# sunhui-3D/3D-PointCloudReconstruction

Measured on NVIDIA B200. Metric: chamfer_fwd_bwd_point_pairs_per_s, higher is better.
Workload: dtype f32

## Files before the change

### 3d-pointcloudreconstruction_b200/_lib.py

```python
import ctypes
import os

import torch

_HERE = os.path.dirname(os.path.abspath(__file__))
LIB_PATH = os.environ.get("PSD_B200_LIB") or os.path.join(_HERE, "libpsd_b200.so")

if not os.path.exists(LIB_PATH):
    raise ImportError(
        f"{LIB_PATH} is missing: build it with `python 3d-pointcloudreconstruction_b200/build.py` "
        "(nvcc, sm_100a). This package has no CPU or eager fallback."
    )

lib = ctypes.CDLL(LIB_PATH)

_vp = ctypes.c_void_p
_ci = ctypes.c_int
_cf = ctypes.c_float

_SIGNATURES = {
    "psd_chamfer_forward": [_vp, _vp, _ci, _ci, _ci, _vp, _vp, _vp, _vp, _vp],
    "psd_chamfer_forward_ex": [_vp, _vp, _ci, _ci, _ci, _ci, _vp, _vp, _vp, _vp, _vp, _cf, _vp, _ci, _ci, _vp],
    "psd_chamfer_forward_zero": [_vp, _vp, _ci, _ci, _ci, _ci, _vp, _vp, _vp, _vp, _vp, _cf, _vp, _vp, ctypes.c_longlong, _vp],
    "psd_chamfer_backward": [_vp] * 8 + [_ci, _ci, _ci, _vp],
# ... 8 lines not shown
    "psd_chamfer_forward_host": [_vp, _vp, _ci, _ci, _ci, _vp, _vp, _vp, _vp, _vp],
    "psd_fp32_fma_peak": [_cf, ctypes.POINTER(_cf), _vp],
    "psd_chamfer_stats": [ctypes.POINTER(ctypes.c_longlong), _ci],
    "psd_chamfer_nn_variant": [_ci],
    "psd_chamfer_mean_loss_forward": [_vp, _vp, _ci, _ci, _ci, _ci, _vp, _vp, _vp, _vp, _vp, _vp, _vp],
    "psd_chamfer_mean_loss_forward_zero": [_vp, _vp, _ci, _ci, _ci, _ci, _vp, _vp, _vp, _vp, _vp, _vp, _vp, ctypes.c_longlong, _vp],
    "psd_chamfer_mean_loss_backward": [_vp, _vp, _vp, _vp, _vp, _vp, _vp, _ci, _ci, _ci, _vp],
    "psd_chamfer_mean_loss_backward_ex": [_vp, _vp, _vp, _vp, _vp, _vp, _vp, _ci, _ci, _ci, _ci, _ci, _vp],
    "psd_chamfer_loss_step_host": [_vp, _vp, _ci, _ci, _ci, _vp, _vp, _vp, _vp, _vp, _vp],
    "psd_chamfer_loss_step_host_ex": [_vp, _vp, _ci, _ci, _ci, _vp, _vp, _vp, _vp, _vp, _ci, _ci, _vp],
    "psd_chamfer_loss_step_pred_dev": [_vp, _ci, _vp, _ci, _ci, _ci, _vp, _vp, _ci, _ci, _vp],
    "psd_host_step_graphs": [_ci],
    "psd_emd_solo_mode": [_ci],
    "psd_emd_grid_mode": [_ci],
    "psd_chamfer_tc_ctas": [_ci],
    "psd_proj_min_dist": [_vp, _vp, _vp, _ci, _ci, _ci, _ci, _vp, _vp, _vp],
    "psd_icp_batch": [_vp, _vp, _ci, _ci, _ci, _vp, _ci, ctypes.c_double, _vp, _vp, _vp, _vp],
    "psd_nn_f64": [_vp, _vp, _ci, _ci, _ci, _ci, _vp, _vp, _vp],
    "psd_farthest_point_sample": [_vp, _ci, _ci, _ci, _ci, _vp, _vp],
    "psd_cont_proj": [_vp, _ci, _ci, _ci, _ci, ctypes.c_float, _vp, _vp],
    "psd_cont_proj_backward": [_vp, _vp, _ci, _ci, _ci, _ci, ctypes.c_float, _vp, _vp],
    "psd_debug_tc_prof": [_vp],
    "psd_debug_tc_filter": [_vp, _vp, _ci, _ci, _ci, _vp, _vp, _vp, _vp, _vp, _ci, _vp],
}
lib.psd_version.restype = _ci
lib.psd_last_error.restype = ctypes.c_char_p
for _n, _a in _SIGNATURES.items():
    getattr(lib, _n).argtypes = _a
    getattr(lib, _n).restype = _ci

# ... 32 lines not shown
```

### 3d-pointcloudreconstruction_b200/csrc/chamfer.cu

```cuda
#include "chamfer_nn.cuh"
#include "psd_device.h"

#ifndef PSD_GRAD_TRIGGER_EARLY
#define PSD_GRAD_TRIGGER_EARLY 1
#endif
namespace psd {

constexpr int kWarps = 16;
constexpr int kThreads = kWarps * 32;
constexpr int kPartBytes = kWarps * kQB * 12;

__device__ unsigned long long g_fallback_queries = 0ull;

struct BlockInfo {
    int blk, d, cloud, qblock;
    float cx, cy, cz;
    float t2max;
    int bad;
    int pad[3];
};
constexpr int kPerBlockBytes = kPartBytes + (int)sizeof(BlockInfo) + 3 * kQB * 4 + kQB * 4;

template <int TM>
__global__ void __launch_bounds__(kThreads, 1) chamfer_nn_kernel(const NNParams p) {
// ... 546 lines not shown
        D.q_bs = 3LL * nq; D.t_bs = 3LL * nt;
        int qb0 = q_begin < 0 ? 0 : q_begin;
        if (qb0 > nq) qb0 = nq;
        int qc = (q_count < 0) ? nq - qb0 : q_count;
        if (qb0 + qc > nq) qc = nq - qb0;
        D.q_begin = qb0; D.q_count = qc;
        D.qblocks = (qc + QB - 1) / QB;
        D.ntt = 1; D.ws = nullptr;
    };
    fill(p.dir[0], xyz1, n, 1, xyz2, m, 2, dist1, idx1, 0);
    fill(p.dir[1], xyz2, m, 2, xyz1, n, 1, dist2, idx2, 1);
    const long long blocks = (long long)b * (p.dir[0].qblocks + p.dir[1].qblocks);
    if (blocks == 0) return only_zero();
    if (blocks > 0x3fffffffLL) return cudaErrorInvalidConfiguration;
    p.zero_buf = zero_buf; p.zero_floats = zero_floats;
    p.pdl_trigger = 0;
    p.blocks_dir0 = b * p.dir[0].qblocks;
    p.total_blocks = (int)blocks;
    p.sums = sums; p.fs_count = fs_count; p.fs_thr = fs_thr;
    p.tile = 0; p.flush = 0;
    const int variant = g_nn_variant.load();
    if ((variant == 3 || (variant == 0 && blocks >= 2LL * num_sms)) && psd_nn_tc_supported(p)) {
        float *dbg = g_tc_dbg.exchange(nullptr);
        return psd_launch_nn_tc(p, ds, stream, dbg, g_tc_dbg_ld.load(), g_tc_prof.load(), b);
    }
    const int grid = blocks < num_sms ? (int)blocks : num_sms;
    const int per_cta = (int)((blocks + grid - 1) / grid);
    int tile = 1024;
    const int tmax = n > m ? n : m;
    while (tile < tmax && tile < 4096) tile *= 2;
    const size_t fixed = (size_t)tile * 16 + 2048;
// ... 70 lines not shown
```

### 3d-pointcloudreconstruction_b200/csrc/chamfer_nn.cuh

```cuda
#pragma once
#include "psd_common.cuh"

namespace psd {

constexpr int kQ = 4;
constexpr int kQB = 32 * kQ;
constexpr int kChunk = 16;
constexpr float kBig = 1e30f;
constexpr float kLimit = 1e18f;
constexpr int kRefTile = 512;

struct NNDirection {
    const float *q;
    const float *t;
    long long q_ps, q_cs, q_bs;
    long long t_ps, t_cs, t_bs;
    float *dist;
    int *idx;
    int nq, nt;
    int q_begin, q_count;
    int qblocks;
    int slot;
    int ntt;
    unsigned long long *ws;
};

struct NNParams {
    NNDirection dir[2];
    int blocks_dir0;
    int total_blocks;
    int tile;
    int flush;
    float *sums;
    int *fs_count;
    float fs_thr;
    float *zero_buf;
    long long zero_floats;
    int pdl_trigger;
};

__device__ __forceinline__ void zero_fill(const NNParams &p) {
    if (p.zero_buf == nullptr) return;
    const long long nth = (long long)gridDim.x * blockDim.x, t0 = (long long)blockIdx.x * blockDim.x + threadIdx.x;
    if (((reinterpret_cast<unsigned long long>(p.zero_buf) & 15ull) == 0ull) && (p.zero_floats & 3) == 0) {
        float4 *z = reinterpret_cast<float4 *>(p.zero_buf);
        for (long long i = t0; i < (p.zero_floats >> 2); i += nth) z[i] = make_float4(0.f, 0.f, 0.f, 0.f);
    } else {
        for (long long i = t0; i < p.zero_floats; i += nth) p.zero_buf[i] = 0.f;
    }
}

__device__ __forceinline__ float exact_d(const float *__restrict__ tb, long long tps, long long tcs, int k, float x1,
                                         float y1, float z1) {
// ... 6 lines not shown
```

### 3d-pointcloudreconstruction_b200/csrc/chamfer_nn_tc.cu

```cuda
#include <cuda_fp16.h>
#include "chamfer_nn.cuh"
#include "psd_device.h"

namespace psd {
namespace tc {

#ifndef PSD_TC_SCAN_WARPS
#define PSD_TC_SCAN_WARPS 8
#endif
#ifndef PSD_TC_SETMAXNREG
#define PSD_TC_SETMAXNREG (PSD_TC_SCAN_WARPS == 16)
#endif
#ifndef PSD_TC_STAGE_FIRST
#define PSD_TC_STAGE_FIRST 0
#endif
#ifndef PSD_TC_TAIL_FAST
#define PSD_TC_TAIL_FAST 1
#endif
#ifndef PSD_TC_ALT_UNROLL
#define PSD_TC_ALT_UNROLL 2
#endif
#ifndef PSD_TC_SCAN_ALT
#define PSD_TC_SCAN_ALT 1
#endif
// ... 23 lines not shown
constexpr int kMaxT = 2048;
constexpr float kPadW = 32768.0f;
constexpr float kQMax = 4096.0f;

constexpr int kOffB = 0;
constexpr int kOffA = kOffB + 2 * kBRows * 32;
constexpr int kOffRaw = kOffA + 2 * kQB * 32;
constexpr int kOffPart = kOffRaw + 2 * 3 * kMaxT * 4;
constexpr int kOffSq = kOffPart + 2 * kColGroups * 3 * kQB * 4;
constexpr int kFbCap = 512;
constexpr int kOffFb = kOffSq + 3 * 3 * kQB * 4;
constexpr int kOffFq = kOffFb + kFbCap * 4;
constexpr int kOffStat = kOffFq + 3 * kFbCap * 4;
constexpr int kOffBar = kOffStat + 3 * 32 * 4 + 16;
constexpr int kOffMisc = kOffBar + 16 * 8;
constexpr int kSmemTC = kOffMisc + 64;
static_assert(kOffBar % 8 == 0 && kOffA % 128 == 0 && kOffRaw % 16 == 0 && kOffPart % 16 == 0 && kHelpWarps <= 8 && kThreadsTC / 32 <= 32 &&
              kSmemTC <= 227 * 1024, "shared-memory carve-up");

__device__ unsigned long long g_fallback_queries_tc = 0ull;

__device__ __forceinline__ uint32_t smem_u32(const void *p) { return (uint32_t)__cvta_generic_to_shared(p); }
__device__ __forceinline__ void mbar_init(uint32_t bar, uint32_t count) {
    asm volatile("mbarrier.init.shared::cta.b64 [%0], %1;" ::"r"(bar), "r"(count) : "memory");
}
__device__ __forceinline__ void mbar_arrive(uint32_t bar) {
    asm volatile("mbarrier.arrive.shared::cta.b64 _, [%0];" ::"r"(bar) : "memory");
}
__device__ __forceinline__ uint32_t mbar_try_wait(uint32_t bar, uint32_t parity) {
    uint32_t ok;
    asm volatile("{ .reg .pred p; mbarrier.try_wait.parity.shared::cta.b64 p, [%1], %2; selp.u32 %0, 1, 0, p; }"
                 : "=r"(ok) : "r"(bar), "r"(parity) : "memory");
    return ok;
// ... 41 lines not shown
        __syncwarp();
    } else if (PSD_TC_SPIN & 2) {
        mbar_spin(bar, parity, abort_flag);
    } else {
        mbar_wait(bar, parity, abort_flag);
    }
}
__device__ __forceinline__ void cp_async4(void *smem_dst, const float *gsrc) {
    asm volatile("cp.async.ca.shared.global [%0], [%1], 4;" ::"r"(smem_u32(smem_dst)), "l"(gsrc) : "memory");
}
__device__ __forceinline__ void cp_async_wait_all() { asm volatile("cp.async.wait_all;" ::: "memory"); }
__device__ __forceinline__ void tc_fence_before() { asm volatile("tcgen05.fence::before_thread_sync;" ::: "memory"); }
__device__ __forceinline__ void tc_fence_after() { asm volatile("tcgen05.fence::after_thread_sync;" ::: "memory"); }
__device__ __forceinline__ void fence_async_smem() { asm volatile("fence.proxy.async.shared::cta;" ::: "memory"); }
__device__ __forceinline__ void help_bar() { asm volatile("bar.sync 1, %0;" ::"n"(kHelpThreads) : "memory"); }
__device__ __forceinline__ void split_h(float x, unsigned short &hi, unsigned short &lo) {
    const __half h = __float2half_rn(x);
    const __half l = __float2half_rn(x - __half2float(h));
    hi = __half_as_ushort(h); lo = __half_as_ushort(l);
}
__device__ __forceinline__ void split_h2(float a, float b, unsigned short &ah, unsigned short &al, unsigned short &bh, unsigned short &bl) {
    const __half2 h = __floats2half2_rn(a, b);
    const float2 hf = __half22float2(h);
    const __half2 l = __floats2half2_rn(a - hf.x, b - hf.y);
    ah = __half_as_ushort(__low2half(h)); bh = __half_as_ushort(__high2half(h));
    al = __half_as_ushort(__low2half(l)); bl = __half_as_ushort(__high2half(l));
}
__device__ __forceinline__ uint32_t pack2(unsigned short a, unsigned short b) { return (uint32_t)a | ((uint32_t)b << 16); }
__device__ __forceinline__ uint64_t umma_desc(uint32_t saddr) {
    return (uint64_t)((saddr & 0x3ffffu) >> 4) | ((uint64_t)(128u >> 4) << 16) | ((uint64_t)(256u >> 4) << 32) |
// ... 77 lines not shown
}
__device__ __forceinline__ int group_of(const NNParams &p, const Unit &u) { return u.d * 0x40000000 + u.cloud * p.dir[u.d].ntt + u.ttile; }
__device__ __forceinline__ const float *targets_of(const NNParams &p, const Unit &u) {
    const NNDirection &D = p.dir[u.d];
    return D.t + (long long)u.cloud * D.t_bs + (long long)u.t0 * D.t_ps;
}
__device__ __forceinline__ void store_result(const NNDirection &D, const Unit &u, int j, float dist, int idx_local) {
    if (D.ws) atomicMin(D.ws + (long long)u.cloud * D.nq + j, pack_key(dist, u.t0 + idx_local));
    else { D.dist[(long long)u.cloud * D.nq + j] = dist; D.idx[(long long)u.cloud * D.nq + j] = u.t0 + idx_local; }
}

struct Frame {
    float cx, cy, cz, cs, wmax;
    int bad, bsel;
};

struct FbQuery {
    Unit u;
    int j, nt, res;
    float x1, y1, z1;
    bool nan_possible;
    const float *bx, *by, *bz;
    long long ps;
};
__device__ __forceinline__ FbQuery fallback_query(const NNParams &p, int blk_begin, int e, const float *sraw, const int *s_rawgroup,
                                                  const float *fq) {
    FbQuery q;
    q.u = decode_unit(p, blk_begin + ((e & 0x3fffffff) >> 8));
    const NNDirection &D = p.dir[q.u.d];
    q.nt = q.u.nt;
// ... 82 lines not shown
    float *sraw = reinterpret_cast<float *>(smem + kOffRaw);
    float *part = reinterpret_cast<float *>(smem + kOffPart);
    float *sq = reinterpret_cast<float *>(smem + kOffSq);
    int *fb_list = reinterpret_cast<int *>(smem + kOffFb);
    float *fb_q = reinterpret_cast<float *>(smem + kOffFq);
    int *s_nfb = reinterpret_cast<int *>(smem + kOffMisc) + 1;
    float *s_wstat = reinterpret_cast<float *>(smem + kOffStat);
    int *s_bstat = reinterpret_cast<int *>(smem + kOffStat) + 32;
    float *s_cstat = reinterpret_cast<float *>(smem + kOffStat) + 64;
    int *s_rawgroup = reinterpret_cast<int *>(smem + kOffStat) + 96;
    uint32_t *s_tmem = reinterpret_cast<uint32_t *>(smem + kOffMisc);
    volatile int *s_abort = reinterpret_cast<volatile int *>(smem + kOffMisc) + 2;
    const uint32_t sB_addr = smem_u32(smem + kOffB), sA_addr = smem_u32(smem + kOffA);
    const uint32_t bar0 = smem_u32(smem + kOffBar);
    const uint32_t bar_full = bar0, bar_empty = bar0 + 8 * kBufs, bar_ready = bar0 + 16 * kBufs, bar_part = bar_ready + 16;

    const int tid = threadIdx.x, lane = tid & 31, warp = tid >> 5;
    const int G = gridDim.x;
    const int blk_begin = (int)(((long long)blockIdx.x * p.total_blocks) / G);
    const int blk_end = (int)(((long long)(blockIdx.x + 1) * p.total_blocks) / G);
    const int nunits = blk_end - blk_begin;
    long long *pf = (DBG && prof) ? prof + (long long)blockIdx.x * 64 : nullptr;
    auto stamp = [&](int slot) { if (DBG && pf && slot < 56) pf[slot] = clock64(); };
    long long *tl = (DBG && prof && blockIdx.x == 0) ? prof + (long long)gridDim.x * 64 : nullptr;
    auto tstamp = [&](int rowi, int g) { if (DBG && tl && g < 64) tl[rowi * 64 + g] = clock64(); };
    if (tid == 0) stamp(0);

    if (tid == 0) {
        for (int i = 0; i < kBufs; ++i) { mbar_init(bar_full + 8 * i, 1); mbar_init(bar_empty + 8 * i, PSD_TC_SCAN_ALT ? 4 : kScanWarps); }
        for (int i = 0; i < 2; ++i) { mbar_init(bar_ready + 8 * i, 1); mbar_init(bar_part + 8 * i, kScanWarps); }
        *s_abort = 0;
        *s_nfb = 0;
        s_rawgroup[0] = -1; s_rawgroup[1] = -1;
        asm volatile("fence.mbarrier_init.release.cluster;" ::: "memory");
    }
    if (warp == kMmaWarp) {
        asm volatile("tcgen05.alloc.cta_group::1.sync.aligned.shared::cta.b32 [%0], %1;" ::"r"(smem_u32(s_tmem)), "r"(512u) : "memory");
        asm volatile("tcgen05.relinquish_alloc_permit.cta_group::1.sync.aligned;" ::: "memory");
    }
    tc_fence_before();
    __syncthreads();
    tc_fence_after();
    const uint32_t tmem_base = *s_tmem;
    if (tid == 0) stamp(1);
    pdl_wait();
    zero_fill(p);

    auto frame_of = [&](int nt, int bsel, int tt, int tn, int tw, auto &&team_bar, Frame &fr, int &bad) {
        const float *rx = sraw + (bsel * 3) * kMaxT, *ry = rx + kMaxT, *rz = ry + kMaxT;
        float cx, cy, cz;
        {
            float sx = 0.f, sy = 0.f, sz = 0.f;
            const int ns = nt < 8 ? nt : 8;
            const int step = nt >> 3;
#pragma unroll
            for (int s8 = 0; s8 < 8; ++s8) {
                if (s8 < ns) {
                    const int k = nt < 8 ? s8 : s8 * step;
// ... 64 lines not shown
    auto build_b = [&](int nt, int bsel, int tt, int tn, int tw, auto &&team_bar, Frame &fr) {
        int bad = 0;
        float wmax = 0.f;
        frame_of(nt, bsel, tt, tn, tw, team_bar, fr, bad);
        build_rows(nt, fr, 0, ((nt + kTileN - 1) / kTileN) * kTileN, tt, tn, wmax, bad);
        publish_stats(tw, wmax, bad);
    };
    auto pick_stats = [&](int nwarps, Frame &fr) {
        float wmax = 0.f;
        int bad = 0;
        for (int w = 0; w < nwarps; ++w) { wmax = fmaxf(wmax, s_wstat[w]); bad |= s_bstat[w]; }
        fr.wmax = wmax; fr.bad = bad;
    };

    Frame fr0 = {0.f, 0.f, 0.f, 1.f, 0.f, 0, 0};
    int group0 = -1;
    float pq1 = 0.f, pq2 = 0.f, pq3 = 0.f;
    if (nunits > 0) {
        const Unit u = decode_unit(p, blk_begin);
        const NNDirection &D = p.dir[u.d];
        group0 = group_of(p, u);
        const float *__restrict__ tb = targets_of(p, u);
#pragma unroll
        for (int comp = 0; comp < 3; ++comp)
            for (int k = tid; k < u.nt; k += kThreadsTC) cp_async4(sraw + comp * kMaxT + k, tb + k * D.t_ps + comp * D.t_cs);
        if (tid >= kHelp0 && tid - kHelp0 < kQB) {
            int j = D.q_begin + u.qblock * kQB + (tid - kHelp0);
            const int q_last = D.q_begin + D.q_count - 1;
            j = j < q_last ? j : q_last;
            const float *qp = D.q + (long long)u.cloud * D.q_bs + j * D.q_ps;
            pq1 = __ldg(qp); pq2 = __ldg(qp + D.q_cs); pq3 = __ldg(qp + 2 * D.q_cs);
        }
        if (tid == 0) stamp(6);
        cp_async_wait_all();
        __syncthreads();
        if (tid == 0) stamp(7);
        build_b(u.nt, 0, tid, kThreadsTC, warp, [] { __syncthreads(); }, fr0);
        fence_async_smem();
        __syncthreads();
        pick_stats(kThreadsTC / 32, fr0);
        if (tid == 0) s_rawgroup[0] = group0;
    }
    if (tid == 0) stamp(5);

    if (warp < kScanWarps) {
        if (PSD_TC_SETMAXNREG) asm volatile("setmaxnreg.dec.sync.aligned.u32 72;");
        const int r = warp & 3, c = warp >> 2;
        const int row = r * 32 + lane;
        const uint32_t tlane = tmem_base + ((uint32_t)(r * 32) << 16);
        int g0 = 0;
        long long a59 = 0;
        Unit u = decode_unit(p, blk_begin);
        for (int ul = 0; ul < nunits; ++ul) {
            if (ul > 0) advance_unit(p, u, blk_begin + ul);
            const int ntiles = (u.nt + kTileN - 1) / kTileN;
// ... 151 lines not shown
                    umma_commit(bar_full + 8 * b);
                    if (DBG) { const long long w3 = clock64(); a61 += w2 - w1; a62 += w3 - w2; if (tl && g < 64) tl[64 + g] = w3; }
                    bdesc += (uint64_t)((kTileN * 32) >> 4);
                }
            }
            if (DBG && pf) { pf[56] = a56; pf[57] = a57; pf[58] = clock64(); pf[61] = a61; pf[62] = a62; }
        }
        __syncwarp();
        if (PSD_TC_SETMAXNREG) asm volatile("setmaxnreg.dec.sync.aligned.u32 80;");
    } else {
        if (PSD_TC_SETMAXNREG) asm volatile("setmaxnreg.inc.sync.aligned.u32 96;");
        const int ht = tid - kHelp0, hw = warp - (kScanWarps + 1);
        int st_group = group0, st_bsel = 0;
        Frame fr_st = fr0;
        bool need_b = false;

        auto stage_changes_group = [&](const Unit &u) { return group_of(p, u) != st_group; };
        auto stage_issue = [&](int ul, const Unit &u) {
            const NNDirection &D = p.dir[u.d];
            if (ht < kQB && ul > 0) {
                int j = D.q_begin + u.qblock * kQB + ht;
                const int q_last = D.q_begin + D.q_count - 1;
                j = j < q_last ? j : q_last;
                const float *qp = D.q + (long long)u.cloud * D.q_bs + j * D.q_ps;
                pq1 = __ldg(qp); pq2 = __ldg(qp + D.q_cs); pq3 = __ldg(qp + 2 * D.q_cs);
            }
            const int group = group_of(p, u);
            need_b = group != st_group;
            if (need_b) {
                st_group = group;
                st_bsel ^= 1;
                const int nt = u.nt;
                const float *__restrict__ tb = targets_of(p, u);
                const long long tps = D.t_ps, tcs = D.t_cs;
                float *rx = sraw + (st_bsel * 3) * kMaxT;
#pragma unroll
                for (int comp = 0; comp < 3; ++comp)
                    for (int k = ht; k < nt; k += kHelpThreads) cp_async4(rx + comp * kMaxT + k, tb + k * tps + comp * tcs);
            }
        };
        auto stage_finish = [&](int ul, const Unit &u) {
            if (need_b) {
                cp_async_wait_all();
                help_bar();
                build_b(u.nt, st_bsel, ht, kHelpThreads, hw, [] { help_bar(); }, fr_st);
                if (ht == 0) s_rawgroup[st_bsel] = st_group;
            }
            if (ht < kQB) {
                float *sqp = sq + (ul % 3) * 3 * kQB;
                sqp[ht] = pq1; sqp[kQB + ht] = pq2; sqp[2 * kQB + ht] = pq3;
                const float sc = -2.0f * fr_st.cs;
                const float x = (pq1 - fr_st.cx) * sc, y = (pq2 - fr_st.cy) * sc, z = (pq3 - fr_st.cz) * sc;
                unsigned short xh, xl, yh, yl, zh, zl, uh, ul_;
                split_h2(x, y, xh, xl, yh, yl);
                split_h2(z, 0.f, zh, zl, uh, ul_);
                const unsigned short one = 0x3c00;
                unsigned char *dst = smem + kOffA + (ul & 1) * (kQB * 32) + (ht >> 3) * 256 + (ht & 7) * 16;
// ... 182 lines not shown
                const FbQuery q = fallback_query(p, blk_begin, fb_list[fi], sraw, s_rawgroup, fb_q + fi);
                const unsigned long long key = fallback_scan(q, item - fi * nsplit, nsplit, lane);
                if (lane == 0) atomicMin(s_keys + fi, key);
            }
            __syncthreads();
            for (int fi = tid; fi < nfb; fi += kThreadsTC) {
                const FbQuery q = fallback_query(p, blk_begin, fb_list[fi], sraw, s_rawgroup, fb_q + fi);
                fallback_write(p, q, s_keys[fi]);
            }
        }
        if (nfb > 0 && tid == 0) atomicAdd(&g_fallback_queries_tc, (unsigned long long)nfb);
    }
    if (tid == 0) stamp(4);
    if (warp == kMmaWarp)
        asm volatile("tcgen05.dealloc.cta_group::1.sync.aligned.b32 %0, %1;" ::"r"(tmem_base), "r"(512u) : "memory");
}

}
}

using namespace psd;

namespace psd {
namespace tc {
__global__ void __launch_bounds__(256) chamfer_nn_tc_finalize_kernel(const NNParams p, int b) {
    const long long n0 = p.dir[0].ws ? (long long)b * p.dir[0].q_count : 0;
    const long long n1 = p.dir[1].ws ? (long long)b * p.dir[1].q_count : 0;
    const long long gid = (long long)blockIdx.x * blockDim.x + threadIdx.x;
    const bool active = gid < n0 + n1;
    const int d = (active && gid >= n0) ? 1 : 0;
// ... 31 lines not shown
            if (p.sums) atomicAdd(p.sums + key2, ws);
            if (p.fs_count && wc) atomicAdd(p.fs_count + key2, wc);
        }
    }
}
}
}

bool psd_nn_tc_supported(const NNParams &p) {
    const long long t0 = (p.dir[0].nt + tc::kMaxT - 1) / tc::kMaxT, t1 = (p.dir[1].nt + tc::kMaxT - 1) / tc::kMaxT;
    return (long long)p.blocks_dir0 * t0 + (long long)(p.total_blocks - p.blocks_dir0) * t1 < 0x3fffffffLL;
}

static std::atomic<int> g_tc_max_ctas{0};
int psd_set_tc_max_ctas(int n) { return n >= 0 ? g_tc_max_ctas.exchange(n) : g_tc_max_ctas.load(); }

static cudaError_t acquire_merge_ws(DeviceState *ds, cudaStream_t stream, size_t elems, unsigned long long **out, bool *temp,
                                    MergeWorkspace **slot_out) {
    *temp = false; *slot_out = nullptr;
    cudaStreamCaptureStatus cap = cudaStreamCaptureStatusNone;
    cudaError_t e = cudaStreamIsCapturing(stream, &cap);
    if (e != cudaSuccess) return e;
    if (cap != cudaStreamCaptureStatusNone) {
        e = cudaMallocAsync(reinterpret_cast<void **>(out), elems * sizeof(unsigned long long), stream);
        if (e == cudaSuccess) e = cudaMemsetAsync(*out, 0xff, elems * sizeof(unsigned long long), stream);
        *temp = true;
        return e;
    }
    std::lock_guard<std::mutex> lock(state_mutex());
    MergeWorkspace *hit = nullptr, *victim = &ds->merge[0];
// ... 19 lines not shown
        if (e != cudaSuccess) { *w = MergeWorkspace(); return e; }
        w->elems = elems;
        w->dirty = true;
    }
    if (w->dirty) {
        e = cudaMemsetAsync(w->ptr, 0xff, w->elems * sizeof(unsigned long long), stream);
        if (e != cudaSuccess) return e;
        w->dirty = false;
    }
    w->used = true; w->stream = stream; w->last_use = ++ds->merge_clock;
    *out = w->ptr; *slot_out = w;
    return cudaSuccess;
}

cudaError_t psd_launch_nn_tc(const NNParams &p_in, DeviceState *ds, cudaStream_t stream, float *dbg, int dbg_ld, long long *prof, int b) {
    {
        std::lock_guard<std::mutex> lock(state_mutex());
        if (!ds->attr_tc) {
            cudaError_t e = cudaFuncSetAttribute(tc::chamfer_nn_tc_kernel<false>, cudaFuncAttributeMaxDynamicSharedMemorySize, tc::kSmemTC);
            if (e == cudaSuccess) e = cudaFuncSetAttribute(tc::chamfer_nn_tc_kernel<true>, cudaFuncAttributeMaxDynamicSharedMemorySize, tc::kSmemTC);
            if (e != cudaSuccess) return e;
            ds->attr_tc = true;
        }
    }
    NNParams p = p_in;
    unsigned long long *ws = nullptr;
    size_t ws_elems = 0;
    bool need_ws[2];
    for (int d = 0; d < 2; ++d) {
        p.dir[d].ntt = (p.dir[d].nt + tc::kMaxT - 1) / tc::kMaxT;
        need_ws[d] = p.dir[d].ntt > 1 && p.dir[d].q_count > 0;
        if (need_ws[d]) ws_elems += (size_t)b * p.dir[d].nq;
    }
    bool ws_temp = false;
    MergeWorkspace *ws_slot = nullptr;
    if (ws_elems) {
        cudaError_t e = acquire_merge_ws(ds, stream, ws_elems, &ws, &ws_temp, &ws_slot);
        if (e != cudaSuccess) return e;
    }
    {
        unsigned long long *w = ws;
        for (int d = 0; d < 2; ++d) {
            p.dir[d].ws = need_ws[d] ? w : nullptr;
            if (need_ws[d]) w += (size_t)b * p.dir[d].nq;
        }
    }
    const int blocks0 = p.blocks_dir0 * p.dir[0].ntt;
    const int blocks1 = (p.total_blocks - p.blocks_dir0) * p.dir[1].ntt;
    p.blocks_dir0 = blocks0;
    p.total_blocks = blocks0 + blocks1;
    int grid = p.total_blocks < ds->num_sms ? p.total_blocks : ds->num_sms;
    const int cap = g_tc_max_ctas.load();
    if (cap > 0 && grid > cap) grid = cap;
    p.pdl_trigger = (cap > 0 && grid == cap) ? 0 : 1;
    cudaError_t e;
    if (dbg || prof) e = psd_launch_pdl(p.pdl_trigger != 0, tc::chamfer_nn_tc_kernel<true>, dim3(grid), dim3(tc::kThreadsTC), tc::kSmemTC, stream, p, dbg, dbg_ld, prof);
    else e = psd_launch_pdl(p.pdl_trigger != 0, tc::chamfer_nn_tc_kernel<false>, dim3(grid), dim3(tc::kThreadsTC), tc::kSmemTC, stream, p, (float *)nullptr, 0, (long long *)nullptr);
    if (ws_elems) {
        if (e == cudaSuccess) {
            const long long total = (p.dir[0].ws ? (long long)b * p.dir[0].q_count : 0) + (p.dir[1].ws ? (long long)b * p.dir[1].q_count : 0);
            if (total > 0) {
                tc::chamfer_nn_tc_finalize_kernel<<<(unsigned)((total + 255) / 256), 256, 0, stream>>>(p, b);
                e = cudaGetLastError();
            }
        }
        if (ws_temp) {
            const cudaError_t e2 = cudaFreeAsync(ws, stream);
            if (e == cudaSuccess) e = e2;
        } else if (e != cudaSuccess && ws_slot) {
            std::lock_guard<std::mutex> lock(state_mutex());
            ws_slot->dirty = true;
        }
// ... 14 lines not shown
```

### 3d-pointcloudreconstruction_b200/csrc/psd_capi.cu

```cuda
#include <stdio.h>
#include <stdlib.h>
#include <string.h>

#include "../../include/psd_b200.h"
#include "psd_common.cuh"
#include "psd_device.h"

cudaError_t psd_launch_chamfer_forward(const float *xyz1, const float *xyz2, int b, int n, int m, int layout,
                                       float *dist1, float *dist2, int *idx1, int *idx2, float *sums, float fs_thr,
                                       int *fs_count, int q_begin, int q_count, cudaStream_t stream, float *zero_buf = nullptr,
                                       long long zero_floats = 0);
cudaError_t psd_launch_chamfer_backward(const float *xyz1, const float *xyz2, float *gradxyz1, float *gradxyz2,
                                        const float *graddist1, const float *graddist2, const int *idx1, const int *idx2,
                                        int b, int n, int m, int layout, int overwrite, cudaStream_t stream,
                                        const float *upstream = nullptr);
cudaError_t psd_launch_chamfer_mean_loss(const float *sums, int b, int n, int m, float *out, cudaStream_t stream);
cudaError_t psd_read_chamfer_stats(unsigned long long *fallback, int reset);
int psd_set_nn_variant(int v);
cudaError_t psd_launch_icp(const void *a, const void *b, int in_f64, int batch, int n, const double *init_pose, int max_iter,
                           double tol, double *T, double *dist, int *iters, cudaStream_t stream);
cudaError_t psd_launch_nn_f64(const void *src, const void *dst, int in_f64, int batch, int n_src, int n_dst, double *distances,
                              int *indices, cudaStream_t stream);
int psd_icp_max_points();
int psd_set_emd_solo(int enable);
int psd_set_emd_grid(int enable);
int psd_set_tc_max_ctas(int n);
cudaError_t psd_launch_cont_proj(const float *pcl, int b, int n, int grid_h, int grid_w, float sigma_sq, float *out,
                                 cudaStream_t stream);
cudaError_t psd_launch_cont_proj_backward(const float *pcl, const float *gout, int b, int n, int grid_h, int grid_w,
                                          float sigma_sq, float *gpcl, cudaStream_t stream);
cudaError_t psd_launch_fps(const float *xyz, int b, int n, int npoint, int start, long long *centroids, cudaStream_t stream);
int psd_fps_max_points();
cudaError_t psd_launch_proj_min_dist(const float *pred, const float *gt, const float *table, int b, int h, int w, int mode,
                                     float *out_min, float *out_inv, cudaStream_t stream);
void psd_set_tc_debug(float *dbg, int ld);
void psd_set_tc_prof(long long *prof);
cudaError_t psd_launch_emd_forward(const float *xyz1, const float *xyz2, int b, int n, float *dist, int *assignment,
                                   float *price, int *assignment_inv, int *bid, float *bid_increments,
                                   float *max_increments, float eps, int iters, int force_cluster, int fresh,
                                   float *loss_sums, cudaStream_t stream, int *unsupported);
cudaError_t psd_launch_emd_mean_loss(const float *sums, int b, int n, float *out, cudaStream_t stream);
// ... 248 lines not shown

int psd_nn_f64(const void *src, const void *dst, int in_f64, int batch, int n_src, int n_dst, double *distances, int *indices,
               void *stream) {
    if (batch < 0 || n_src < 0 || n_dst < 1) { psd_set_error_msg("psd_nn_f64: batch >= 0, n_src >= 0, n_dst >= 1 required"); return -1; }
    if ((size_t)n_dst * 24 > 200 * 1024) { psd_set_error_msg("psd_nn_f64: destination cloud too large for shared memory (n_dst <= 8533)"); return -1; }
    return finish("psd_nn_f64", psd_launch_nn_f64(src, dst, in_f64, batch, n_src, n_dst, distances, indices, (cudaStream_t)stream));
}

int psd_chamfer_nn_variant(int variant) { return psd_set_nn_variant(variant); }

int psd_emd_solo_mode(int enable) { return psd_set_emd_solo(enable); }

int psd_emd_grid_mode(int enable) { return psd_set_emd_grid(enable); }

int psd_chamfer_tc_ctas(int max_ctas) { return psd_set_tc_max_ctas(max_ctas); }

int psd_debug_tc_prof(long long *prof_dev) { psd_set_tc_prof(prof_dev); return 1; }

int psd_debug_tc_filter(const float *xyz1, const float *xyz2, int b, int n, int m, float *dist1, float *dist2, int *idx1,
                        int *idx2, float *dump, int dump_ld, void *stream) {
    const int old = psd_set_nn_variant(3);
    psd_set_tc_debug(dump, dump_ld);
    cudaError_t e = psd_launch_chamfer_forward(xyz1, xyz2, b, n, m, 0, dist1, dist2, idx1, idx2, nullptr, 0.f, nullptr, 0,
                                               -1, (cudaStream_t)stream);
    psd_set_tc_debug(nullptr, 0);
    psd_set_nn_variant(old);
    return finish("psd_debug_tc_filter", e);
}

int psd_chamfer_stats(long long *out_host2, int reset) {
// ... 73 lines not shown
    const bool own_g1 = (g1 == d_g1);
    if (!own_g1 && (e = cudaMemsetAsync(g1, 0, sizeof(float) * 3 * s1, stream)) != cudaSuccess) return e;
    e = psd_launch_chamfer_forward(x1, d_x2, b, n, m, layout, d_d1, d_d2, d_i1, d_i2, d_sums, 0.f, nullptr, 0, -1, stream,
                                   own_g1 ? d_g1 : d_g2, (long long)(own_g1 ? 3 * (s1 + s2) : 3 * s2));
    if (e == cudaSuccess) e = psd_launch_chamfer_mean_loss(d_sums, b, n, m, d_loss, stream);
    if (e == cudaSuccess) e = psd_launch_chamfer_backward(x1, d_x2, g1, d_g2, nullptr, nullptr, d_i1, d_i2, b, n, m, layout, 0, stream, nullptr);
    if (e != cudaSuccess) return e;
    e = cudaMemcpyAsync(a.loss_host, d_loss, sizeof(float), cudaMemcpyDeviceToHost, stream);
    if (e == cudaSuccess && a.g1_host) e = cudaMemcpyAsync(a.g1_host, g1, sizeof(float) * 3 * s1, cudaMemcpyDeviceToHost, stream);
    if (e == cudaSuccess && a.g2_host) e = cudaMemcpyAsync(a.g2_host, d_g2, sizeof(float) * 3 * s2, cudaMemcpyDeviceToHost, stream);
    return e;
}

struct StepGraph {
    const void *x1 = nullptr, *x2 = nullptr, *loss = nullptr, *g1 = nullptr, *g2 = nullptr, *g1u = nullptr, *ws = nullptr;
    int b = 0, n = 0, m = 0, variant = 0, device = -1, tc_ctas = 0, flags = 0;
    cudaGraphExec_t exec = nullptr;
    bool plain = false;
    unsigned long long last_use = 0;
    bool same(const StepGraph &o) const {
        return x1 == o.x1 && x2 == o.x2 && loss == o.loss && g1 == o.g1 && g2 == o.g2 && g1u == o.g1u && ws == o.ws && b == o.b &&
               n == o.n && m == o.m && variant == o.variant && device == o.device && tc_ctas == o.tc_ctas && flags == o.flags;
    }
};
static const int kStepGraphs = 64;
static StepGraph g_step_graph[kStepGraphs];
static unsigned long long g_step_clock = 0;
static int g_step_graph_enabled = -1;

static void drop_step_graphs(const void *ws) {
    for (StepGraph &g : g_step_graph)
        if (g.ws == ws) {
            if (g.exec) cudaGraphExecDestroy(g.exec);
            g = StepGraph();
        }
}

// ... 30 lines not shown
        ds->step_ws_bytes[slot] = need;
    }
    float *const ws = ds->step_ws[slot];
    if (gradxyz1_dev) *gradxyz1_dev = (a.x1_dev && a.g1_user) ? a.g1_user : ws + 3 * (s1 + s2);
    if (gradxyz2_dev) *gradxyz2_dev = ws + 3 * (s1 + s2) + 3 * s1;

    if (g_step_graph_enabled < 0) {
        const char *env = getenv("PSD_HOST_STEP_GRAPH");
        g_step_graph_enabled = (env && env[0] == '0') ? 0 : 1;
    }
    bool launched = false;
    if (g_step_graph_enabled && stream != nullptr && stream != cudaStreamLegacy) {
        StepGraph key;
        key.x1 = a.x1; key.x2 = a.x2; key.loss = a.loss_host; key.g1 = a.g1_host; key.g2 = a.g2_host; key.g1u = a.g1_user;
        key.ws = ws; key.b = b; key.n = n; key.m = m; key.variant = psd_set_nn_variant(-1); key.tc_ctas = psd_set_tc_max_ctas(-1);
        key.flags = (a.x1_dev ? 1 : 0) | (a.layout1 ? 2 : 0);
        key.device = ds->device;
        StepGraph *hit = nullptr, *victim = &g_step_graph[0];
        for (StepGraph &g : g_step_graph) {
            if (g.ws && g.same(key)) { hit = &g; break; }
            if (g.last_use < victim->last_use) victim = &g;
        }
        if (hit == nullptr) {
            if (victim->exec) cudaGraphExecDestroy(victim->exec);
            *victim = key;
            victim->last_use = ++g_step_clock;
        } else {
            hit->last_use = ++g_step_clock;
            if (hit->exec == nullptr && !hit->plain &&
                !((a.x1_dev || pinned_host(a.x1)) && pinned_host(a.x2) && pinned_host(a.loss_host) && pinned_host(a.g1_host) &&
// ... 113 lines not shown
```

### 3d-pointcloudreconstruction_b200/csrc/psd_common.cuh

```cuda
#pragma once
#include <cuda_runtime.h>
#include <stdint.h>

#if defined(__CUDA_ARCH__) && (__CUDA_ARCH__ < 1000)
#error "libpsd_b200 is written for sm_100a (B200) only"
#endif

namespace psd {

__device__ __forceinline__ float sqdist_exact(float dx, float dy, float dz) {
    return __fmaf_rn(dz, dz, __fmaf_rn(dx, dx, __fmul_rn(dy, dy)));
}

__device__ __forceinline__ float2 ffma2(float a, float2 b, float2 c) {
    return __ffma2_rn(make_float2(a, a), b, c);
}

__device__ __forceinline__ float fmin3(float a, float b, float c) {
    float d;
    asm("min.f32 %0, %1, %2, %3;" : "=f"(d) : "f"(a), "f"(b), "f"(c));
    return d;
}

#ifndef PSD_PDL
// ... 5 lines not shown
__device__ __forceinline__ void pdl_wait() {
    if (PSD_PDL) asm volatile("griddepcontrol.wait;" ::: "memory");
}

__device__ __forceinline__ unsigned long long pack_key(float d, int idx) {
    return ((unsigned long long)__float_as_uint(d) << 32) | (unsigned int)idx;
}

__device__ __forceinline__ unsigned long long shfl_xor_u64(unsigned long long v, int lane_mask) {
    return __shfl_xor_sync(0xffffffffu, v, lane_mask);
}

}

template <typename... KArgs, typename... Args>
static inline cudaError_t psd_launch_pdl(bool allow, void (*kernel)(KArgs...), dim3 grid, dim3 block, size_t smem, cudaStream_t stream, Args... args) {
    cudaLaunchConfig_t cfg = {};
    cfg.gridDim = grid; cfg.blockDim = block; cfg.dynamicSmemBytes = smem; cfg.stream = stream;
    cudaLaunchAttribute at[1];
    at[0].id = cudaLaunchAttributeProgrammaticStreamSerialization;
    at[0].val.programmaticStreamSerializationAllowed = (PSD_PDL && allow) ? 1 : 0;
    cfg.attrs = at; cfg.numAttrs = 1;
    return cudaLaunchKernelEx(&cfg, kernel, KArgs(args)...);
}

void psd_set_error(const char *what, cudaError_t err);
void psd_set_error_msg(const char *what);
```

### 3d-pointcloudreconstruction_b200/csrc/psd_device.h

```cpp
#pragma once
#include <cuda_runtime.h>

#include <atomic>
#include <mutex>

namespace psd {

constexpr int kMaxDevices = 64;
constexpr int kStepSlots = 8;
constexpr int kMergeSlots = 16;

struct MergeWorkspace {
    cudaStream_t stream = nullptr;
    unsigned long long *ptr = nullptr;
    size_t elems = 0;
    bool used = false;
    bool dirty = false;
    unsigned long long last_use = 0;
};

struct DeviceState {
    bool init = false;
    int device = -1;
    int num_sms = 0, max_smem = 0;
    bool attr_nn = false, attr_tc = false, attr_proj = false;
    float *fwd_ws = nullptr;
    size_t fwd_ws_bytes = 0;
    float *step_ws[kStepSlots] = {};
    size_t step_ws_bytes[kStepSlots] = {};
    MergeWorkspace merge[kMergeSlots];
    unsigned long long merge_clock = 0;
};

DeviceState *device_state(cudaError_t *err);
std::mutex &state_mutex();

}
```

### include/psd_b200.h

```cpp
#ifndef PSD_B200_H_
#define PSD_B200_H_

#ifdef __cplusplus
extern "C" {
#endif

int psd_version(void);

const char *psd_last_error(void);


int psd_chamfer_forward(const float *xyz1, const float *xyz2, int b, int n, int m, float *dist1, float *dist2,
                        int *idx1, int *idx2, void *stream);

int psd_chamfer_forward_ex(const float *xyz1, const float *xyz2, int b, int n, int m, int layout, float *dist1,
                           float *dist2, int *idx1, int *idx2, float *sums, float fs_thr, int *fs_count, int q_begin,
                           int q_count, void *stream);

int psd_chamfer_forward_zero(const float *xyz1, const float *xyz2, int b, int n, int m, int layout, float *dist1,
                             float *dist2, int *idx1, int *idx2, float *sums, float fs_thr, int *fs_count, float *zero_buf,
                             long long zero_floats, void *stream);

int psd_chamfer_backward(const float *xyz1, const float *xyz2, float *gradxyz1, float *gradxyz2,
                         const float *graddist1, const float *graddist2, const int *idx1, const int *idx2, int b, int n,
// ... 61 lines not shown
                                  int slot, int sync, void *stream);
int psd_chamfer_loss_step_pred_dev(const float *xyz1_dev, int layout1, const float *xyz2_host, int b, int n, int m,
                                   float *loss_host, float *gradxyz1_dev, int slot, int sync, void *stream);
int psd_host_step_graphs(int enable);


int psd_fp32_fma_peak(float ms_target, float *tflops, void *stream);

int psd_chamfer_stats(long long *out_host2, int reset);

int psd_chamfer_nn_variant(int variant);

int psd_emd_solo_mode(int enable);
int psd_emd_grid_mode(int enable);
int psd_chamfer_tc_ctas(int max_ctas);

int psd_debug_tc_filter(const float *xyz1, const float *xyz2, int b, int n, int m, float *dist1, float *dist2, int *idx1,
                        int *idx2, float *dump, int dump_ld, void *stream);

int psd_debug_tc_prof(long long *prof_dev);

#ifdef __cplusplus
}
#endif
#endif
```

Before: 7122 billion.

## Share target-tile B-operand builds between paired CTAs via 2-CTA clusters and DSMEM

Launches the tensor-core chamfer kernel as 2-CTA clusters. When a pair of CTAs each need the same two target groups at a group boundary, each CTA builds one group's split-half B operand and bulk-copies it, together with its frame, into the peer's shared memory through DSMEM with mbarrier transaction tracking. This is meant to remove duplicated target loads and B-operand construction at the start of each CTA's work range. In exchange it adds cluster barriers, a remote-arrive handshake before exit, and a cluster launch constraint that could limit occupancy. Pairing is on by default when the grid is even and enough clusters fit.

```diff
diff --git a/3d-pointcloudreconstruction_b200/_lib.py b/3d-pointcloudreconstruction_b200/_lib.py
--- a/3d-pointcloudreconstruction_b200/_lib.py
+++ b/3d-pointcloudreconstruction_b200/_lib.py
@@ -46,6 +46,7 @@
     "psd_emd_solo_mode": [_ci],
     "psd_emd_grid_mode": [_ci],
     "psd_chamfer_tc_ctas": [_ci],
+    "psd_chamfer_tc_pairs": [_ci],
     "psd_proj_min_dist": [_vp, _vp, _vp, _ci, _ci, _ci, _ci, _vp, _vp, _vp],
     "psd_icp_batch": [_vp, _vp, _ci, _ci, _ci, _vp, _ci, ctypes.c_double, _vp, _vp, _vp, _vp],
     "psd_nn_f64": [_vp, _vp, _ci, _ci, _ci, _ci, _vp, _vp, _vp],
diff --git a/3d-pointcloudreconstruction_b200/csrc/chamfer.cu b/3d-pointcloudreconstruction_b200/csrc/chamfer.cu
--- a/3d-pointcloudreconstruction_b200/csrc/chamfer.cu
+++ b/3d-pointcloudreconstruction_b200/csrc/chamfer.cu
@@ -584,7 +584,7 @@
     if (blocks == 0) return only_zero();
     if (blocks > 0x3fffffffLL) return cudaErrorInvalidConfiguration;
     p.zero_buf = zero_buf; p.zero_floats = zero_floats;
-    p.pdl_trigger = 0;
+    p.pdl_trigger = 0; p.pairs = 0;
     p.blocks_dir0 = b * p.dir[0].qblocks;
     p.total_blocks = (int)blocks;
     p.sums = sums; p.fs_count = fs_count; p.fs_thr = fs_thr;
diff --git a/3d-pointcloudreconstruction_b200/csrc/chamfer_nn.cuh b/3d-pointcloudreconstruction_b200/csrc/chamfer_nn.cuh
--- a/3d-pointcloudreconstruction_b200/csrc/chamfer_nn.cuh
+++ b/3d-pointcloudreconstruction_b200/csrc/chamfer_nn.cuh
@@ -37,6 +37,7 @@
     float *zero_buf;
     long long zero_floats;
     int pdl_trigger;
+    int pairs;
 };
 
 __device__ __forceinline__ void zero_fill(const NNParams &p) {
diff --git a/3d-pointcloudreconstruction_b200/csrc/chamfer_nn_tc.cu b/3d-pointcloudreconstruction_b200/csrc/chamfer_nn_tc.cu
--- a/3d-pointcloudreconstruction_b200/csrc/chamfer_nn_tc.cu
+++ b/3d-pointcloudreconstruction_b200/csrc/chamfer_nn_tc.cu
@@ -61,9 +61,10 @@
 constexpr int kOffStat = kOffFq + 3 * kFbCap * 4;
 constexpr int kOffBar = kOffStat + 3 * 32 * 4 + 16;
 constexpr int kOffMisc = kOffBar + 16 * 8;
+constexpr int kOffXFrame = kOffMisc + 16;
 constexpr int kSmemTC = kOffMisc + 64;
-static_assert(kOffBar % 8 == 0 && kOffA % 128 == 0 && kOffRaw % 16 == 0 && kOffPart % 16 == 0 && kHelpWarps <= 8 && kThreadsTC / 32 <= 32 &&
-              kSmemTC <= 227 * 1024, "shared-memory carve-up");
+static_assert(kOffBar % 8 == 0 && kOffA % 128 == 0 && kOffRaw % 16 == 0 && kOffPart % 16 == 0 && kOffXFrame % 16 == 0 &&
+              kHelpWarps <= 8 && kThreadsTC / 32 <= 32 && kSmemTC <= 227 * 1024, "shared-memory carve-up");
 
 __device__ unsigned long long g_fallback_queries_tc = 0ull;
 
@@ -135,6 +136,28 @@
 __device__ __forceinline__ void tc_fence_after() { asm volatile("tcgen05.fence::after_thread_sync;" ::: "memory"); }
 __device__ __forceinline__ void fence_async_smem() { asm volatile("fence.proxy.async.shared::cta;" ::: "memory"); }
 __device__ __forceinline__ void help_bar() { asm volatile("bar.sync 1, %0;" ::"n"(kHelpThreads) : "memory"); }
+__device__ __forceinline__ uint32_t cluster_rank() {
+    uint32_t r;
+    asm volatile("mov.u32 %0, %%cluster_ctarank;" : "=r"(r));
+    return r;
+}
+__device__ __forceinline__ uint32_t map_to_rank(uint32_t saddr, uint32_t rank) {
+    uint32_t r;
+    asm volatile("mapa.shared::cluster.u32 %0, %1, %2;" : "=r"(r) : "r"(saddr), "r"(rank));
+    return r;
+}
+__device__ __forceinline__ void cluster_arrive() { asm volatile("barrier.cluster.arrive.relaxed.aligned;" ::: "memory"); }
+__device__ __forceinline__ void cluster_wait() { asm volatile("barrier.cluster.wait.acquire.aligned;" ::: "memory"); }
+__device__ __forceinline__ void mbar_arrive_remote(uint32_t cluster_bar) {
+    asm volatile("mbarrier.arrive.release.cluster.shared::cluster.b64 _, [%0];" ::"r"(cluster_bar) : "memory");
+}
+__device__ __forceinline__ void mbar_expect_tx(uint32_t bar, uint32_t bytes) {
+    asm volatile("mbarrier.arrive.expect_tx.shared::cta.b64 _, [%0], %1;" ::"r"(bar), "r"(bytes) : "memory");
+}
+__device__ __forceinline__ void bulk_copy_to_cluster(uint32_t dst, uint32_t src, uint32_t bytes, uint32_t bar) {
+    asm volatile("cp.async.bulk.shared::cluster.shared::cta.mbarrier::complete_tx::bytes [%0], [%1], %2, [%3];"
+                 ::"r"(dst), "r"(src), "r"(bytes), "r"(bar) : "memory");
+}
 __device__ __forceinline__ void split_h(float x, unsigned short &hi, unsigned short &lo) {
     const __half h = __float2half_rn(x);
     const __half l = __float2half_rn(x - __half2float(h));
@@ -242,6 +265,34 @@
     float cx, cy, cz, cs, wmax;
     int bad, bsel;
 };
+
+struct PairPlan {
+    int role;
+    int buf;
+    int blk1;
+    uint32_t bytes;
+};
+__device__ __forceinline__ PairPlan pair_plan(const NNParams &p) {
+    PairPlan pl = {0, 0, 0, 0u};
+    if (!p.pairs) return pl;
+    const long long G = gridDim.x, lo = blockIdx.x & ~1u;
+    const int b0 = (int)((lo * p.total_blocks) / G), b1 = (int)(((lo + 1) * p.total_blocks) / G),
+              b2 = (int)(((lo + 2) * p.total_blocks) / G);
+    if (b0 == b1 || b1 == b2) return pl;
+    const Unit u0 = decode_unit(p, b0);
+    const int e1 = b0 + p.dir[u0.d].qblocks - u0.qblock;
+    if (e1 >= b2 || e1 == b1) return pl;
+    const Unit u1 = decode_unit(p, e1);
+    if (e1 + p.dir[u1.d].qblocks < b2) return pl;
+    const bool upper = (blockIdx.x & 1) != 0, lower_crosses = e1 < b1;
+    pl.role = upper == lower_crosses ? 1 : 2;
+    pl.buf = lower_crosses ? 1 : 0;
+    pl.blk1 = e1;
+    const int nt = lower_crosses ? u1.nt : u0.nt;
+    pl.bytes = (uint32_t)(((nt + kTileN - 1) / kTileN) * kTileN * 32 + 32);
+    return pl;
+}
+static_assert(sizeof(Frame) <= 32, "Frame slot");
 
 struct FbQuery {
     Unit u;
@@ -354,6 +405,9 @@
     const uint32_t sB_addr = smem_u32(smem + kOffB), sA_addr = smem_u32(smem + kOffA);
     const uint32_t bar0 = smem_u32(smem + kOffBar);
     const uint32_t bar_full = bar0, bar_empty = bar0 + 8 * kBufs, bar_ready = bar0 + 16 * kBufs, bar_part = bar_ready + 16;
+    const uint32_t bar_xfer = bar_part + 16;
+    const uint32_t bar_done = bar_xfer + 8;
+    Frame *s_xframe = reinterpret_cast<Frame *>(smem + kOffXFrame);
 
     const int tid = threadIdx.x, lane = tid & 31, warp = tid >> 5;
     const int G = gridDim.x;
@@ -365,10 +419,14 @@
     long long *tl = (DBG && prof && blockIdx.x == 0) ? prof + (long long)gridDim.x * 64 : nullptr;
     auto tstamp = [&](int rowi, int g) { if (DBG && tl && g < 64) tl[rowi * 64 + g] = clock64(); };
     if (tid == 0) stamp(0);
+    const PairPlan pl = pair_plan(p);
+    if (DBG && pf && tid == 0) pf[63] = pl.role + 4 * pl.buf;
 
     if (tid == 0) {
         for (int i = 0; i < kBufs; ++i) { mbar_init(bar_full + 8 * i, 1); mbar_init(bar_empty + 8 * i, PSD_TC_SCAN_ALT ? 4 : kScanWarps); }
         for (int i = 0; i < 2; ++i) { mbar_init(bar_ready + 8 * i, 1); mbar_init(bar_part + 8 * i, kScanWarps); }
+        if (pl.role == 2) { mbar_init(bar_xfer, 1); mbar_expect_tx(bar_xfer, pl.bytes); }
+        if (pl.role == 1) mbar_init(bar_done, 1);
         *s_abort = 0;
         *s_nfb = 0;
         s_rawgroup[0] = -1; s_rawgroup[1] = -1;
@@ -382,6 +440,7 @@
     __syncthreads();
     tc_fence_after();
     const uint32_t tmem_base = *s_tmem;
+    if (pl.role != 0) cluster_arrive();
     if (tid == 0) stamp(1);
     pdl_wait();
     zero_fill(p);
@@ -476,6 +535,8 @@
     };
 
     Frame fr0 = {0.f, 0.f, 0.f, 1.f, 0.f, 0, 0};
+    Frame fr_b1 = fr0;
+    const bool build_g1 = pl.role == 2 && pl.buf == 0;
     int group0 = -1;
     float pq1 = 0.f, pq2 = 0.f, pq3 = 0.f;
     if (nunits > 0) {
@@ -486,6 +547,14 @@
 #pragma unroll
         for (int comp = 0; comp < 3; ++comp)
             for (int k = tid; k < u.nt; k += kThreadsTC) cp_async4(sraw + comp * kMaxT + k, tb + k * D.t_ps + comp * D.t_cs);
+        const Unit u1 = build_g1 ? decode_unit(p, pl.blk1) : u;
+        if (build_g1) {
+            const NNDirection &D1 = p.dir[u1.d];
+            const float *__restrict__ tb1 = targets_of(p, u1);
+#pragma unroll
+            for (int comp = 0; comp < 3; ++comp)
+                for (int k = tid; k < u1.nt; k += kThreadsTC) cp_async4(sraw + (3 + comp) * kMaxT + k, tb1 + k * D1.t_ps + comp * D1.t_cs);
+        }
         if (tid >= kHelp0 && tid - kHelp0 < kQB) {
             int j = D.q_begin + u.qblock * kQB + (tid - kHelp0);
             const int q_last = D.q_begin + D.q_count - 1;
@@ -497,10 +566,29 @@
         cp_async_wait_all();
         __syncthreads();
         if (tid == 0) stamp(7);
-        build_b(u.nt, 0, tid, kThreadsTC, warp, [] { __syncthreads(); }, fr0);
+        Frame fr;
+        build_b(build_g1 ? u1.nt : u.nt, build_g1 ? 1 : 0, tid, kThreadsTC, warp, [] { __syncthreads(); }, fr);
         fence_async_smem();
         __syncthreads();
-        pick_stats(kThreadsTC / 32, fr0);
+        pick_stats(kThreadsTC / 32, fr);
+        if (pl.role != 0) cluster_wait();
+        if (build_g1) {
+            fr_b1 = fr;
+            if (tid == 0) s_rawgroup[1] = group_of(p, u1);
+            mbar_wait(bar_xfer, 0, s_abort);
+            if (tid == 0) mbar_arrive_remote(map_to_rank(bar_done, cluster_rank() ^ 1u));
+            fr0 = *s_xframe;
+            fr0.bsel = 0;
+        } else {
+            fr0 = fr;
+            if (pl.role == 1 && tid == 0) {
+                *s_xframe = fr0;
+                fence_async_smem();
+                const uint32_t peer = cluster_rank() ^ 1u, peer_bar = map_to_rank(bar_xfer, peer);
+                bulk_copy_to_cluster(map_to_rank(sB_addr + (uint32_t)pl.buf * (kBRows * 32), peer), sB_addr, pl.bytes - 32, peer_bar);
+                bulk_copy_to_cluster(map_to_rank(smem_u32(s_xframe), peer), smem_u32(s_xframe), 32, peer_bar);
+            }
+        }
         if (tid == 0) s_rawgroup[0] = group0;
     }
     if (tid == 0) stamp(5);
@@ -682,6 +770,7 @@
         int st_group = group0, st_bsel = 0;
         Frame fr_st = fr0;
         bool need_b = false;
+        const int group_b1 = pl.role == 2 ? group_of(p, decode_unit(p, pl.blk1)) : -1;
 
         auto stage_changes_group = [&](const Unit &u) { return group_of(p, u) != st_group; };
         auto stage_issue = [&](int ul, const Unit &u) {
@@ -698,6 +787,7 @@
             if (need_b) {
                 st_group = group;
                 st_bsel ^= 1;
+                if (build_g1 && group == group_b1) return;
                 const int nt = u.nt;
                 const float *__restrict__ tb = targets_of(p, u);
                 const long long tps = D.t_ps, tcs = D.t_cs;
@@ -708,7 +798,18 @@
             }
         };
         auto stage_finish = [&](int ul, const Unit &u) {
-            if (need_b) {
+            if (need_b && st_group == group_b1) {
+                if (build_g1) {
+                    fr_st = fr_b1;
+                } else {
+                    cp_async_wait_all();
+                    mbar_wait_warp(bar_xfer, 0, s_abort);
+                    if (ht == 0) mbar_arrive_remote(map_to_rank(bar_done, cluster_rank() ^ 1u));
+                    fr_st = *s_xframe;
+                    fr_st.bsel = st_bsel;
+                    if (ht == 0) s_rawgroup[st_bsel] = st_group;
+                }
+            } else if (need_b) {
                 cp_async_wait_all();
                 help_bar();
                 build_b(u.nt, st_bsel, ht, kHelpThreads, hw, [] { help_bar(); }, fr_st);
@@ -921,6 +1022,7 @@
     if (tid == 0) stamp(4);
     if (warp == kMmaWarp)
         asm volatile("tcgen05.dealloc.cta_group::1.sync.aligned.b32 %0, %1;" ::"r"(tmem_base), "r"(512u) : "memory");
+    if (pl.role == 1 && tid == 0) mbar_wait(bar_done, 0, s_abort);
 }
 
 }
@@ -982,6 +1084,8 @@
 
 static std::atomic<int> g_tc_max_ctas{0};
 int psd_set_tc_max_ctas(int n) { return n >= 0 ? g_tc_max_ctas.exchange(n) : g_tc_max_ctas.load(); }
+static std::atomic<int> g_tc_pairs{1};
+int psd_set_tc_pairs(int enable) { return (enable == 0 || enable == 1) ? g_tc_pairs.exchange(enable) : g_tc_pairs.load(); }
 
 static cudaError_t acquire_merge_ws(DeviceState *ds, cudaStream_t stream, size_t elems, unsigned long long **out, bool *temp,
                                     MergeWorkspace **slot_out) {
@@ -1031,14 +1135,26 @@
 }
 
 cudaError_t psd_launch_nn_tc(const NNParams &p_in, DeviceState *ds, cudaStream_t stream, float *dbg, int dbg_ld, long long *prof, int b) {
+    int pair_clusters;
     {
         std::lock_guard<std::mutex> lock(state_mutex());
         if (!ds->attr_tc) {
             cudaError_t e = cudaFuncSetAttribute(tc::chamfer_nn_tc_kernel<false>, cudaFuncAttributeMaxDynamicSharedMemorySize, tc::kSmemTC);
             if (e == cudaSuccess) e = cudaFuncSetAttribute(tc::chamfer_nn_tc_kernel<true>, cudaFuncAttributeMaxDynamicSharedMemorySize, tc::kSmemTC);
+            cudaLaunchConfig_t cfg = {};
+            cfg.gridDim = dim3(2); cfg.blockDim = dim3(tc::kThreadsTC); cfg.dynamicSmemBytes = tc::kSmemTC;
+            cudaLaunchAttribute at[1];
+            at[0].id = cudaLaunchAttributeClusterDimension;
+            at[0].val.clusterDim.x = 2; at[0].val.clusterDim.y = 1; at[0].val.clusterDim.z = 1;
+            cfg.attrs = at; cfg.numAttrs = 1;
+            int n0 = 0, n1 = 0;
+            if (e == cudaSuccess) e = cudaOccupancyMaxActiveClusters(&n0, tc::chamfer_nn_tc_kernel<false>, &cfg);
+            if (e == cudaSuccess) e = cudaOccupancyMaxActiveClusters(&n1, tc::chamfer_nn_tc_kernel<true>, &cfg);
             if (e != cudaSuccess) return e;
+            ds->tc_pair_clusters = n0 < n1 ? n0 : n1;
             ds->attr_tc = true;
         }
+        pair_clusters = ds->tc_pair_clusters;
     }
     NNParams p = p_in;
     unsigned long long *ws = nullptr;
@@ -1069,10 +1185,13 @@
     int grid = p.total_blocks < ds->num_sms ? p.total_blocks : ds->num_sms;
     const int cap = g_tc_max_ctas.load();
     if (cap > 0 && grid > cap) grid = cap;
-    p.pdl_trigger = (cap > 0 && grid == cap) ? 0 : 1;
+    const bool capped = cap > 0 && grid == cap;
+    p.pdl_trigger = capped ? 0 : 1;
+    p.pairs = (g_tc_pairs.load() && !capped && grid % 2 == 0 && pair_clusters >= grid / 2) ? 1 : 0;
+    const int cluster = p.pairs ? 2 : 1;
     cudaError_t e;
-    if (dbg || prof) e = psd_launch_pdl(p.pdl_trigger != 0, tc::chamfer_nn_tc_kernel<true>, dim3(grid), dim3(tc::kThreadsTC), tc::kSmemTC, stream, p, dbg, dbg_ld, prof);
-    else e = psd_launch_pdl(p.pdl_trigger != 0, tc::chamfer_nn_tc_kernel<false>, dim3(grid), dim3(tc::kThreadsTC), tc::kSmemTC, stream, p, (float *)nullptr, 0, (long long *)nullptr);
+    if (dbg || prof) e = psd_launch_pdl(p.pdl_trigger != 0, cluster, tc::chamfer_nn_tc_kernel<true>, dim3(grid), dim3(tc::kThreadsTC), tc::kSmemTC, stream, p, dbg, dbg_ld, prof);
+    else e = psd_launch_pdl(p.pdl_trigger != 0, cluster, tc::chamfer_nn_tc_kernel<false>, dim3(grid), dim3(tc::kThreadsTC), tc::kSmemTC, stream, p, (float *)nullptr, 0, (long long *)nullptr);
     if (ws_elems) {
         if (e == cudaSuccess) {
             const long long total = (p.dir[0].ws ? (long long)b * p.dir[0].q_count : 0) + (p.dir[1].ws ? (long long)b * p.dir[1].q_count : 0);
diff --git a/3d-pointcloudreconstruction_b200/csrc/psd_capi.cu b/3d-pointcloudreconstruction_b200/csrc/psd_capi.cu
--- a/3d-pointcloudreconstruction_b200/csrc/psd_capi.cu
+++ b/3d-pointcloudreconstruction_b200/csrc/psd_capi.cu
@@ -25,6 +25,7 @@
 int psd_set_emd_solo(int enable);
 int psd_set_emd_grid(int enable);
 int psd_set_tc_max_ctas(int n);
+int psd_set_tc_pairs(int enable);
 cudaError_t psd_launch_cont_proj(const float *pcl, int b, int n, int grid_h, int grid_w, float sigma_sq, float *out,
                                  cudaStream_t stream);
 cudaError_t psd_launch_cont_proj_backward(const float *pcl, const float *gout, int b, int n, int grid_h, int grid_w,
@@ -303,6 +304,8 @@
 int psd_emd_grid_mode(int enable) { return psd_set_emd_grid(enable); }
 
 int psd_chamfer_tc_ctas(int max_ctas) { return psd_set_tc_max_ctas(max_ctas); }
+
+int psd_chamfer_tc_pairs(int enable) { return psd_set_tc_pairs(enable); }
 
 int psd_debug_tc_prof(long long *prof_dev) { psd_set_tc_prof(prof_dev); return 1; }
 
@@ -406,13 +409,13 @@
 
 struct StepGraph {
     const void *x1 = nullptr, *x2 = nullptr, *loss = nullptr, *g1 = nullptr, *g2 = nullptr, *g1u = nullptr, *ws = nullptr;
-    int b = 0, n = 0, m = 0, variant = 0, device = -1, tc_ctas = 0, flags = 0;
+    int b = 0, n = 0, m = 0, variant = 0, device = -1, tc_ctas = 0, tc_pairs = 0, flags = 0;
     cudaGraphExec_t exec = nullptr;
     bool plain = false;
     unsigned long long last_use = 0;
     bool same(const StepGraph &o) const {
         return x1 == o.x1 && x2 == o.x2 && loss == o.loss && g1 == o.g1 && g2 == o.g2 && g1u == o.g1u && ws == o.ws && b == o.b &&
-               n == o.n && m == o.m && variant == o.variant && device == o.device && tc_ctas == o.tc_ctas && flags == o.flags;
+               n == o.n && m == o.m && variant == o.variant && device == o.device && tc_ctas == o.tc_ctas && tc_pairs == o.tc_pairs && flags == o.flags;
     }
 };
 static const int kStepGraphs = 64;
@@ -473,6 +476,7 @@
         StepGraph key;
         key.x1 = a.x1; key.x2 = a.x2; key.loss = a.loss_host; key.g1 = a.g1_host; key.g2 = a.g2_host; key.g1u = a.g1_user;
         key.ws = ws; key.b = b; key.n = n; key.m = m; key.variant = psd_set_nn_variant(-1); key.tc_ctas = psd_set_tc_max_ctas(-1);
+        key.tc_pairs = psd_set_tc_pairs(-1);
         key.flags = (a.x1_dev ? 1 : 0) | (a.layout1 ? 2 : 0);
         key.device = ds->device;
         StepGraph *hit = nullptr, *victim = &g_step_graph[0];
diff --git a/3d-pointcloudreconstruction_b200/csrc/psd_common.cuh b/3d-pointcloudreconstruction_b200/csrc/psd_common.cuh
--- a/3d-pointcloudreconstruction_b200/csrc/psd_common.cuh
+++ b/3d-pointcloudreconstruction_b200/csrc/psd_common.cuh
@@ -43,13 +43,15 @@
 }
 
 template <typename... KArgs, typename... Args>
-static inline cudaError_t psd_launch_pdl(bool allow, void (*kernel)(KArgs...), dim3 grid, dim3 block, size_t smem, cudaStream_t stream, Args... args) {
+static inline cudaError_t psd_launch_pdl(bool allow, int cluster, void (*kernel)(KArgs...), dim3 grid, dim3 block, size_t smem, cudaStream_t stream, Args... args) {
     cudaLaunchConfig_t cfg = {};
     cfg.gridDim = grid; cfg.blockDim = block; cfg.dynamicSmemBytes = smem; cfg.stream = stream;
-    cudaLaunchAttribute at[1];
+    cudaLaunchAttribute at[2];
     at[0].id = cudaLaunchAttributeProgrammaticStreamSerialization;
     at[0].val.programmaticStreamSerializationAllowed = (PSD_PDL && allow) ? 1 : 0;
-    cfg.attrs = at; cfg.numAttrs = 1;
+    at[1].id = cudaLaunchAttributeClusterDimension;
+    at[1].val.clusterDim.x = (unsigned)cluster; at[1].val.clusterDim.y = 1; at[1].val.clusterDim.z = 1;
+    cfg.attrs = at; cfg.numAttrs = cluster > 1 ? 2 : 1;
     return cudaLaunchKernelEx(&cfg, kernel, KArgs(args)...);
 }
 
diff --git a/3d-pointcloudreconstruction_b200/csrc/psd_device.h b/3d-pointcloudreconstruction_b200/csrc/psd_device.h
--- a/3d-pointcloudreconstruction_b200/csrc/psd_device.h
+++ b/3d-pointcloudreconstruction_b200/csrc/psd_device.h
@@ -24,6 +24,7 @@
     int device = -1;
     int num_sms = 0, max_smem = 0;
     bool attr_nn = false, attr_tc = false, attr_proj = false;
+    int tc_pair_clusters = 0;
     float *fwd_ws = nullptr;
     size_t fwd_ws_bytes = 0;
     float *step_ws[kStepSlots] = {};
diff --git a/include/psd_b200.h b/include/psd_b200.h
--- a/include/psd_b200.h
+++ b/include/psd_b200.h
@@ -99,6 +99,7 @@
 int psd_emd_solo_mode(int enable);
 int psd_emd_grid_mode(int enable);
 int psd_chamfer_tc_ctas(int max_ctas);
+int psd_chamfer_tc_pairs(int enable);
 
 int psd_debug_tc_filter(const float *xyz1, const float *xyz2, int b, int n, int m, float *dist1, float *dist2, int *idx1,
                         int *idx2, float *dump, int dump_ld, void *stream);
```

Result: slower. 7003 billion (median of 6 runs) (-1.7%).
